# orybkin/video-gcp

Measured on AMD Instinct MI355X. Metric: predicted frames/sec, 64x64x3 seq_len=80 gcp_tree (posterior forward + all loss terms, model(inputs) and model.loss() of train.py:157-159, batch-stat BatchNorm), higher is better.
Workload: dtype f32 (encoder / decoder convs and the tree GEMMs from 512 rows: split-f16 MFMA with f32 accumulate, f32-equivalent; everything else exact f32 MFMA)

## Files before the change

### include/gcpx.h

```cpp
#ifndef GCPX_H
#define GCPX_H

#include <stdint.h>

#ifdef __cplusplus
extern "C" {
#endif

#define GCPX_VERSION 1

typedef enum gcpx_status {
    GCPX_OK = 0,
    GCPX_ERR_INVALID_ARG = -1,
    GCPX_ERR_UNSUPPORTED = -2,
    GCPX_ERR_HIP = -3,
    GCPX_ERR_COMM = -4
} gcpx_status;

typedef enum gcpx_act { GCPX_ACT_NONE = 0, GCPX_ACT_LRELU = 1, GCPX_ACT_TANH = 2 } gcpx_act;

int gcpx_version(void);
const char* gcpx_last_error(void);
int gcpx_conv_grid(void);

// ... 16 lines not shown
    GCPX_HEAD_DLM_NLL_GRAD = 5
} gcpx_head_mode;

typedef struct gcpx_conv_args {
    gcpx_conv_src src[2];
    int32_t nsrc;
    int32_t F;
    int32_t Hin, Win;
    int32_t Hout, Wout;
    int32_t Cin;
    int32_t Cout;
    int32_t out_pitch;
    int32_t upsample;
    int32_t out_act;
    int32_t head_mode;
    const float* wpk;
    const float* bias;
    float* out;
    float* images;
    float* stats_partial;
    const int32_t* raw_row_map;
    const int32_t* src_row_map;
    const int32_t* src_row_frames;
    int32_t n_src_rows;
    int32_t w_split_log2;
    const void* wpk_split;
    const int32_t* w_split_log2_dev;
    int32_t split_layout;
    int32_t nll_rows;
    const float* nll_target;
    float* nll_partial;
    const float* nll_row_weight;
    float nll_scale;
    int32_t _pad3;
    float* images_rows;
    int64_t images_rows_dup;
    const float* bwd_r;
    const float *bwd_scale, *bwd_shift, *bwd_mean, *bwd_rstd;
    const float* addend;
    int32_t addend_frame_div;
    int32_t _pad4;
} gcpx_conv_args;

typedef enum gcpx_split_layout { GCPX_SPLIT_PLAIN = 0, GCPX_SPLIT_ROWFOLD = 1, GCPX_SPLIT_HEAD32 = 2, GCPX_SPLIT_ROWFOLD16 = 3,
                                 GCPX_SPLIT_LOWRES = 4 } gcpx_split_layout;

int gcpx_conv3x3(const gcpx_conv_args* a, void* stream);
int gcpx_conv3x3_grid(const gcpx_conv_args* a);
int gcpx_conv3x3_lowres_supported(const gcpx_conv_args* a);
int gcpx_conv4x4s2(const gcpx_conv_args* a, void* stream);
int gcpx_conv4x4s2_grid(void);
int gcpx_conv4x4s2_image(const float* x, const float* wpk, const float* bias, float* out,
                         int32_t F, int32_t Hin, int32_t Win, int32_t Cout, int32_t out_act, void* stream);

int gcpx_bn_finalize(const float* partial, int32_t n_partial, int32_t pitch, int32_t C, double count,
                     const float* gamma, const float* beta, float eps, float* scale, float* shift,
                     float* running_mean, float* running_var, float momentum, float* mean_out, float* rstd_out,
                     void* stream);
int gcpx_randn(float* out, int64_t n, uint64_t* state, void* stream);
int gcpx_bn_fold(const float* running_mean, const float* running_var, const float* gamma, const float* beta,
                 float eps, int32_t C, float* scale, float* shift, void* stream);

typedef struct gcpx_row_src {
    const float* ptr;
    const int32_t* rowidx;
    const float* scale;
    const float* shiftv;
    int64_t sb, sr;
    int32_t width;
    int32_t shift;
    int32_t act;
    int32_t cmod;
} gcpx_row_src;

typedef enum gcpx_gemm_epi {
    GCPX_EPI_NONE = 0,
    GCPX_EPI_LRELU = 1,
    GCPX_EPI_LSTM = 2,
    GCPX_EPI_GAUSS_SAMPLE = 3
} gcpx_gemm_epi;

struct gcpx_lstm_bwd_args;
typedef struct gcpx_gemm_args {
    gcpx_row_src src[6];
    int32_t nsrc;
    int32_t M, N, K, rpb;
    const float* wpk;
    const float* bias;
    float* out;
    int64_t ob, orow;
    int32_t epi;
    int32_t nbatch;
    float* stats_partial;
    const float* c_prev;
    int64_t c_prev_stride;
    float* h_out;
    float* c_out;
    int64_t hb, hrow;
    float* h_copy;
    int64_t z_src_off, z_w_off, z_bias_off, z_out_off;
    float* gates_out;
    const void* wpk_split;
    const int32_t* w_split_log2_dev;
    int32_t w_split_log2;
    int32_t _pad_split;
    void* x_planes;
// ... 541 lines not shown
```

### video-gcp_amd/forward_plan.py

```python
import ctypes as C
import os
from contextlib import contextmanager

import torch

from . import packing as pk
from . import runtime as rt
from .hparams import GCPHParams
from .params import init_params, encoder_layers, encoder_skip_layers, decoder_layers
from .plan_ops import _Plan, _addr, N_LANES


class ForwardPlanMixin:

    def _plan_encoder(self, plan, tag, x_ptr, F, out_ptr, out_ob, out_orow, out_rpb):
        hp, P, lib = self._hp, self.pk, self.lib
        G = lib.gcpx_conv4x4s2_grid()
        S = hp.img_sz
        skip_idx = encoder_skip_layers(hp)
        skips = {}
        a0 = self._buf(f"{tag}.a0", (F, S // 2, S // 2, hp.ngf))
        enc_rec = dict(F=F, x_ptr=x_ptr, a0=a0, r={}, out=(out_ptr, out_ob, out_orow, out_rpb))
        plan.rec[f"enc:{tag}"] = enc_rec
        plan.add(f"enc.input:{tag}", lib.gcpx_conv4x4s2_image, x_ptr, P["enc.input.w"].data_ptr(),
                 P["enc.input.b"].data_ptr(), a0.data_ptr(), F, S, S, hp.ngf, rt.ACT_LRELU)
        prev = (a0.data_ptr(), hp.ngf, 1, None, None, rt.ACT_NONE)
        if 0 in skip_idx:
            skips[0] = (a0, hp.ngf, None, None, rt.ACT_NONE)
        res = S // 2
        for li, (name, cin, cout, norm) in enumerate(self._enc_layers[1:], start=1):
            r = self._buf(f"{tag}.r{li}", (F, res // 2, res // 2, cout))
            enc_rec["r"][li] = r
            stats = self._buf(f"{tag}.st{li}", (G, 2, cout)) if self.training else None
            a = self._conv_args([prev], F, res, res, res // 2, res // 2, cout, cout, P[f"enc.{name}.w"],
                                P[f"enc.{name}.b"], r, stats=stats)
            self._set_split(a, f"enc.{name}")
            plan.keep.append(a)
            plan.add(f"enc.{name}:{tag}", lib.gcpx_conv4x4s2, C.byref(a))
            res //= 2
            scale, shift = self._bn(plan, f"{tag}.bn{li}", f"encoder.net.{name}.norm", cout, stats, G, cout,
                                    F * res * res)
            prev = (r.data_ptr(), cout, 1, scale, shift, rt.ACT_LRELU)
            if li in skip_idx:
                skips[li] = (r, cout, scale, shift, rt.ACT_LRELU)
        assert res == 4
        ctop = self._c_top
        src = self._rowsrc(prev[0], 16 * ctop, 16 * ctop, 16 * ctop, scale=prev[3], shiftv=prev[4], act=prev[5], cmod=ctop)
        src.sb, src.sr = out_rpb * 16 * ctop, 16 * ctop
        self._gemm(plan, f"enc.head:{tag}", [src], F, hp.nz_enc, out_rpb, P["enc.head.w"], P["enc.head.b"],
                   out=out_ptr, ob=out_ob, orow=out_orow)
        return skips

    def _plan_seq_encoder(self, plan, tag, prefix, enc_traj, out, B):
        hp, P, lib = self._hp, self.pk, self.lib
        T, nz = hp.max_seq_len, hp.nz_enc
        y1 = self._buf(f"{tag}.y1", (B * T, hp.nz_mid))
        y2 = self._buf(f"{tag}.y2", (B * T, hp.nz_mid))
        taps = lambda t, w, **kw: [self._rowsrc(t.data_ptr(), T * w, w, w, shift=d, **kw) for d in (-1, 0, 1)]
        self._gemm(plan, f"{tag}.input", taps(enc_traj, nz), B * T, hp.nz_mid, T, P[f"{tag}.input.w"], P[f"{tag}.input.b"],
                   out=y1.data_ptr(), ob=T * hp.nz_mid, orow=hp.nz_mid, epi=rt.EPI_LRELU)
        assert hp.conv_inf_enc_layers == 1
        nrb = lib.gcpx_gemm_row_blocks(B * T, hp.nz_mid)
        st = self._buf(f"{tag}.st", (nrb, 2, hp.nz_mid)) if self.training else None
        self._gemm(plan, f"{tag}.pyramid-0", taps(y1, hp.nz_mid), B * T, hp.nz_mid, T, P[f"{tag}.pyramid-0.w"],
                   P[f"{tag}.pyramid-0.b"], out=y2.data_ptr(), ob=T * hp.nz_mid, orow=hp.nz_mid, stats=st)
        sc, sh = self._bn(plan, f"{tag}.bn", f"{prefix}.net.pyramid-0.norm", hp.nz_mid, st, nrb, hp.nz_mid, B * T)
        self._gemm(plan, f"{tag}.head", taps(y2, hp.nz_mid, scale=sc, shiftv=sh, act=rt.ACT_LRELU, cmod=hp.nz_mid),
                   B * T, nz, T, P[f"{tag}.head.w"], P[f"{tag}.head.b"], out=out.data_ptr(), ob=T * nz, orow=nz)

    def _plan_attention(self, plan, l, W, el, er, M, n, B, Kp, Vp, tin):
        hp, lib = self._hp, self.lib
        T, nz, dk = hp.max_seq_len, hp.nz_enc, hp.nz_attn_key
        li = l if hp.untied_layers else 0
        qin = self._buf(f"attn.qin{l}", (M, dk))
        self._mlp(plan, f"attn.query{l}", W["attn.query"], [el, er], M, n, out=qin.data_ptr(), ob=n * dk, orow=dk)
        dense = lambda t, w: self._rowsrc(t.data_ptr(), 0, w, w)
        qp = self._buf(f"attn.q{l}", (M, dk))
        self._gemm(plan, f"attn.q_proj{l}", [dense(qin, dk)], M, dk, M, W["attn.q_proj.w"], W["attn.q_proj.b"],
                   out=qp.data_ptr(), ob=0, orow=dk)
        o = self._buf(f"attn.o{l}", (M, nz))
        gamma = self._buf(f"attn.gamma{l}", (M, T))
        temp = self.sd[f"tree_module.tree_modules.{li}.inference.attention.attention_layers.0.temperature"]
        plan.add(f"attn{l}", lib.gcpx_attention, qp.data_ptr(), _addr(Kp, li * B * T * dk), _addr(Vp, li * B * T * nz), None,
                 tin["end_ind"].data_ptr(), temp.data_ptr(), o.data_ptr(), gamma.data_ptr(), M, n, T, dk, nz, hp.n_attention_heads)
        raw = self._buf(f"attn.raw{l}", (M, nz))
        self._gemm(plan, f"attn.out_proj{l}", [dense(o, nz)], M, nz, M, W["attn.out_proj.w"], W["attn.out_proj.b"],
                   out=raw.data_ptr(), ob=0, orow=nz)
        et = self._buf(f"attn.e_tilde{l}", (M, nz))
        self._gemm(plan, f"attn.out{l}", [dense(raw, nz)], M, nz, M, W["attn.out.w"], W["attn.out.b"], out=et.data_ptr(), ob=0, orow=nz)
        plan.rec.setdefault("gamma", {})[l] = gamma
        plan.rec.setdefault("e_tilde", {})[l] = et
# ... 64 lines not shown
    def _build_plan(self, key, tin):
        hp, P, lib = self._hp, self.pk, self.lib
        B, has_traj, has_z, sample_prior, phase, pred_len = key.B, key.has_traj, key.has_z, key.sample_prior, key.phase, key.pred_len
        train_aux = has_traj and phase == "train" and not sample_prior
        L, T, N = hp.hierarchy_levels, hp.max_seq_len, hp.n_nodes
        nz, nv, H, SD = hp.nz_enc, hp.nz_vae, hp.nz_mid_lstm, hp.lstm_state_dim
        PS = 2 ** L + 1
        plan = _Plan(lib)
        G = lib.gcpx_conv_grid()
        def plan_aux_indices():
            AUXK = ("inv_t0", "inv_t1", "cost_start_idx", "cost_end_idx")
            plan.add("aux_sample_indices", lib.gcpx_aux_sample_indices_gauss, tin["end_ind"].data_ptr(), tin["aux_n"].data_ptr(), B,
                     hp.inv_mdl_temp_dist, *[tin[k].data_ptr() for k in AUXK])
        if "aux_n" in tin and pred_len:
            plan_aux_indices()

        E = self._buf("E", (B, PS, nz))
        Hid = self._buf("Hid", (B, PS, SD))
        Z = self._buf("Z", (B, PS, nv))
        PZ = self._buf("PZ", (B, PS, 2 * nv))
        QZ = self._buf("QZ", (B, PS, 2 * nv))
        node_t = self._buf("node_t", (B, N), torch.int32)
        leave = self._buf("leave", (B, N), torch.int32)
        f2n = self._buf("frame2node", (B, T), torch.int32)
        etrow = self._buf("etilde_row", (B * N,), torch.int32)
        seq_len = self._buf("seq_len", (B,), torch.int32)
        kept_idx = self._buf("kept_idx", (B, T), torch.int32)
        node2row = self._buf("node2row", (B, N), torch.int32)

        adaptive, attentive = hp.adaptive, hp.attentive_inference
        if adaptive:
            kept_idx = self._buf("kept_idx", (B, N), torch.int32)
        def plan_bookkeeping():
            if not adaptive:
                plan.add("balanced_binding", lib.gcpx_balanced_binding, tin["end_ind"].data_ptr(), B, L, T, node_t.data_ptr(),
                         leave.data_ptr(), f2n.data_ptr(), etrow.data_ptr(), seq_len.data_ptr(), node2row.data_ptr())
                plan.add("compact_index", lib.gcpx_compact_index, leave.data_ptr(), B, N, T, kept_idx.data_ptr())
                r2f = self._buf("row2frame", (B * T,), torch.int32)
                if self._head_grad_fused(key) or self._rows_direct(key):
                    plan.add("row2frame", lib.gcpx_index_inverse, node2row.data_ptr(), B * N, r2f.data_ptr(), B * T)
                if self._head_grad_fused(key):
                    S_ = hp.img_sz
                    dMD = self._buf("bw.dMD", (B * T, S_, S_, self._head_pitch))
                    plan.add("zero_unmapped", lib.gcpx_zero_unmapped_rows, dMD.data_ptr(), S_ * S_ * self._head_pitch, r2f.data_ptr(), B * T)

        enc_traj = inf_enc = None
        plan.fork([1, 2])
        traj_first = os.environ.get("GCPX_ENC_ORDER") != "small_first"
        def plan_traj_encoder():
            nonlocal enc_traj, inf_enc
            plan.lane = 0
            if has_traj:
                enc_traj = self._buf("enc_traj", (B * T, nz))
                self._plan_encoder(plan, "traj", tin["traj_seq"].data_ptr(), B * T, enc_traj.data_ptr(), T * nz, nz, T)
                if hp.seq_enc == "none":
                    inf_enc = enc_traj
                else:
                    inf_enc = self._buf("inf_enc_seq", (B * T, nz))
                    self._plan_seq_encoder(plan, "seq", "inf_encoder", enc_traj, inf_enc, B)
                if attentive:
                    dk = hp.nz_attn_key
                    n_mod = L if hp.untied_layers else 1
                    if hp.seq_enc == "none":
                        kenc = enc_traj
                    else:
                        kenc = self._buf("inf_key_enc", (B * T, nz))
                        self._plan_seq_encoder(plan, "kseq", "inf_key_encoder.0", enc_traj, kenc, B)
                    keys = self._buf("inf_enc_key_seq", (B * T, dk))
                    dense = lambda t, w: self._rowsrc(t.data_ptr(), 0, w, w)
                    self._gemm(plan, "kseq.key", [dense(kenc, nz)], B * T, dk, B * T, P["kseq.key.w"], P["kseq.key.b"],
                               out=keys.data_ptr(), ob=0, orow=dk)
                    Kp = self._buf("attn.K", (n_mod, B * T, dk))
                    Vp = self._buf("attn.V", (n_mod, B * T, nz))
                    self._gemm(plan, "attn.k_proj", [dense(keys, dk)], B * T, dk, B * T, P["attn.k_proj.w"], P["attn.k_proj.b"],
                               out=Kp.data_ptr(), ob=0, orow=dk, batch=(n_mod, 0, P["attn.k_proj.w"][0].numel(), dk, B * T * dk))
                    self._gemm(plan, "attn.v_proj", [dense(inf_enc, nz)], B * T, nz, B * T, P["attn.v_proj.w"], P["attn.v_proj.b"],
                               out=Vp.data_ptr(), ob=0, orow=nz, batch=(n_mod, 0, P["attn.v_proj.w"][0].numel(), nz, B * T * nz))
                    plan.rec["attn_kv"] = dict(Kp=Kp, Vp=Vp, keys=keys, kenc=kenc, n_mod=n_mod)

        if traj_first:
            plan_traj_encoder()
        plan.lane = 1
        if "rng_all" in tin:
            plan.add("randn", lib.gcpx_randn, tin["rng_all"].data_ptr(), tin["rng_all"].numel(), self._buf("rng_state", (2,), torch.int64).data_ptr())
            if "aux_n" in tin and not pred_len:
                plan.wait(2, 1)
        skips = self._plan_encoder(plan, "I0", tin["I_0"].data_ptr(), B, _addr(E), PS * nz, 0, 1)
        plan.lane = 2
        if not pred_len:
            if "aux_n" in tin:
                plan_aux_indices()
            plan_bookkeeping()
        if hp.attach_cost_mdl and hp.run_cost_mdl and train_aux and self._has_aux_training:
            gt = self._buf("cost_target", (B,))
            rows = hp.input_nc * hp.img_sz
            plan.add("path_cost", lib.gcpx_path_cost, tin["traj_seq"].data_ptr(), tin["cost_start_idx"].data_ptr(),
                     tin["cost_end_idx"].data_ptr(), B, T, rows, hp.img_sz, self._buf("cost_partial", (B, rows)).data_ptr(), gt.data_ptr())
        self._plan_encoder(plan, "Ig", tin["I_g"].data_ptr(), B, _addr(E, 2 ** L * nz), PS * nz, 0, 1)
        outs = {}
        e0 = lambda: self._rowsrc(_addr(E), PS * nz, 0, nz)
        eg = lambda: self._rowsrc(_addr(E, 2 ** L * nz), PS * nz, 0, nz)
        if hp.regress_length and not pred_len:
            plan.wait(2, 1)
            logits = self._buf("seq_len_logits", (B, T))
            self._mlp(plan, "length_pred", P["length_pred"], [e0(), eg()], B, 1, out=logits.data_ptr(), ob=T, orow=0)
            outs["seq_len_logits"] = logits
        if not traj_first:
            plan_traj_encoder()
        plan.lane = 0
        plan.join([1, 2])

        if hp.regress_length and pred_len:
            logits = self._buf("seq_len_logits", (B, T))
            self._mlp(plan, "length_pred", P["length_pred"], [e0(), eg()], B, 1, out=logits.data_ptr(), ob=T, orow=0)
            outs["seq_len_logits"] = logits
            plan.add("sample_length", lib.gcpx_sample_length, logits.data_ptr(), tin["len_u"].data_ptr(), B, T, 2, tin["end_ind"].data_ptr())
            plan_bookkeeping()

        side_merge = False
        for l in range(L):
            W = P[f"tree{l if hp.untied_layers else 0}"]
            s = 2 ** (L - 1 - l)
            n = 2 ** l
            M = B * n
            nodeoff = lambda w: s * w
            el = lambda: self._rowsrc(_addr(E), PS * nz, 2 * s * nz, nz)
            er = lambda: self._rowsrc(_addr(E, 2 * s * nz), PS * nz, 2 * s * nz, nz)
            pz_out = (_addr(PZ, nodeoff(2 * nv)), PS * 2 * nv, 2 * s * 2 * nv)
            z_map = (_addr(Z, nodeoff(nv)), PS * nv, 2 * s * nv)
            nl = hp.n_lstm_layers
            merged = self._buf(f"merged{l}", (M, 2 * nl * H))

            def plan_merge(lv=l, group=None):
                s_, n_ = 2 ** (L - 1 - lv), 2 ** lv
                Wl = P[f"tree{lv if hp.untied_layers else 0}"]
                mg = self._buf(f"merged{lv}", (B * n_, 2 * nl * H))
                if hp.tree_lstm == "sum":
                    for side, mode in ((0, 0), (2 * s_ * SD, 1)):
                        plan.add(f"merge{lv}.{mode}", lib.gcpx_rows_strided, _addr(mg), n_ * SD, SD, _addr(Hid, side), PS * SD, 2 * s_ * SD,
                                 B, n_, SD, mode)
                    return
                if hp.tree_lstm == "linear":
                    h1 = self._rowsrc(_addr(Hid), PS * SD, 2 * s_ * SD, SD)
                    h2 = self._rowsrc(_addr(Hid, 2 * s_ * SD), PS * SD, 2 * s_ * SD, SD)
                    self._gemm(plan, f"merge{lv}", [h1, h2], B * n_, SD, n_, Wl["proj.w"], Wl["proj.b"], out=_addr(mg), ob=n_ * SD, orow=SD,
                               group=group)
                    return
                h1 = self._rowsrc(_addr(Hid), PS * SD, 2 * s_ * SD, H)
                h2 = self._rowsrc(_addr(Hid, 2 * s_ * SD), PS * SD, 2 * s_ * SD, H)
                self._gemm(plan, f"merge{lv}", [h1, h2], B * n_, H, n_, Wl["proj.w"], Wl["proj.b"], out=_addr(mg),
                           ob=n_ * 2 * nl * H, orow=2 * nl * H, batch=(2 * nl, H, Wl["proj.w"][0].numel(), H, H), group=group)
# ... 319 lines not shown
```

### video-gcp_amd/runtime.py

```python
import ctypes as C
import os

_HERE = os.path.dirname(os.path.abspath(__file__))
LIB_PATH = os.path.join(_HERE, "libgcpx.so")

ACT_NONE, ACT_LRELU, ACT_TANH = 0, 1, 2
HEAD_RAW, HEAD_DLM_MEAN, HEAD_DLM_BOTH, HEAD_TANH_NCHW, HEAD_DLM_NLL, HEAD_DLM_NLL_GRAD = 0, 1, 2, 3, 4, 5
SPLIT_PLAIN, SPLIT_ROWFOLD, SPLIT_HEAD32, SPLIT_ROWFOLD16, SPLIT_LOWRES = 0, 1, 2, 3, 4
EPI_NONE, EPI_LRELU, EPI_LSTM, EPI_GAUSS_SAMPLE = 0, 1, 2, 3
GEMM_FORM_TILE, GEMM_FORM_SPLIT_K, GEMM_FORM_SPLIT_F16, GEMM_FORM_PLANES = 0, 1, 2, 3
MLP_PLAIN, MLP_GAUSS, MLP_TANH = 0, 1, 2

vp = C.c_void_p
i32 = C.c_int32
i64 = C.c_int64


class ConvSrc(C.Structure):
    _fields_ = [("ptr", vp), ("scale", vp), ("shift", vp), ("C", i32), ("frame_div", i32), ("act", i32), ("_pad", i32)]


class ConvArgs(C.Structure):
    _fields_ = [("src", ConvSrc * 2), ("nsrc", i32), ("F", i32), ("Hin", i32), ("Win", i32), ("Hout", i32),
                ("Wout", i32), ("Cin", i32), ("Cout", i32), ("out_pitch", i32), ("upsample", i32), ("out_act", i32),
# ... 61 lines not shown

class LstmBwdArgs(C.Structure):
    _fields_ = [("gates", vp), ("c_prev", vp), ("c_new", vp), ("dh_dense", vp), ("dh_pos", vp), ("dc_pos", vp),
                ("dgates", vp), ("dc_prev", vp), ("c_prev_stride", i64), ("pb", i64), ("prow", i64), ("dh_stride", i64),
                ("dcp_stride", i64), ("M", i32), ("H", i32), ("rpb", i32), ("_pad", i32)]


class TreeAccumSrc(C.Structure):
    _fields_ = [("ptr", vp), ("ld", i64), ("off_left", i32), ("off_right", i32), ("off_ctx0", i32), ("off_ctxg", i32),
                ("dst_col", i32), ("_pad", i32)]


class TreeAccumArgs(C.Structure):
    _fields_ = [("src", TreeAccumSrc * 6), ("dst", vp), ("dst_sb", i64), ("slot_stride", i64), ("nsrc", i32), ("B", i32),
                ("n", i32), ("width", i32)]


class ActBwdArgs(C.Structure):
    _fields_ = [("da", vp), ("add", vp), ("r", vp), ("scale", vp), ("shift", vp), ("mean", vp), ("rstd", vp), ("dy", vp),
                ("stats_partial", vp), ("ldc", i64), ("c_off", i32), ("up", i32), ("fsum", i32), ("act", i32), ("F", i32),
                ("H", i32), ("W", i32), ("C", i32)]


class PanelTile(C.Structure):
    _fields_ = [("kind", i32), ("src", i32), ("index", i32), ("length", i32), ("flags", i32), ("nb", i32), ("nf", i32),
                ("h", i32), ("w", i32), ("tile_w", i32), ("n0", i32), ("n_b", i32), ("n_f", i32), ("r0", i32), ("r_b", i32),
                ("r_f", i32), ("c0", i32), ("c_b", i32), ("c_f", i32), ("index_off", i32), ("index_stride", i32),
                ("index_count", i32), ("fill", C.c_float), ("_pad", i32), ("off", i64), ("s_b", i64), ("s_f", i64), ("s_c", i64),
                ("s_y", i64)]


class TrajLayer(C.Structure):
    _fields_ = [("states", vp), ("s_n", i64), ("s_p", i64), ("s_d", i64), ("len", vp), ("dim_t", vp), ("color", C.c_float * 3),
                ("len_i64", i32), ("K", i32), ("P", i32)]


PANEL_MAX_SRCS = 16
PANEL_IMAGE, PANEL_GREY, PANEL_GREY_ADD, PANEL_FILL = 0, 1, 2, 3
PANEL_RESCALE, PANEL_LENGTH_STRICT, PANEL_INDEX_FRAME, PANEL_INDEX_I64, PANEL_LENGTH_I64 = 1, 2, 4, 8, 16

WG_ROWS, WG_CONV1D, WG_CONV3X3, WG_CONV4X4S2 = 0, 1, 2, 3
WMAP_LINEAR, WMAP_CONV, WMAP_CONVT = 0, 1, 2

SYMBOLS = [
    ("gcpx_version", C.c_int, []),
    ("gcpx_last_error", C.c_char_p, []),
    ("gcpx_conv_grid", C.c_int, []),
    ("gcpx_conv3x3", C.c_int, [C.POINTER(ConvArgs), vp]),
    ("gcpx_conv3x3_grid", C.c_int, [C.POINTER(ConvArgs)]),
    ("gcpx_conv3x3_lowres_supported", C.c_int, [C.POINTER(ConvArgs)]),
    ("gcpx_conv4x4s2", C.c_int, [C.POINTER(ConvArgs), vp]),
    ("gcpx_conv4x4s2_grid", C.c_int, []),
    ("gcpx_conv4x4s2_image", C.c_int, [vp, vp, vp, vp, i32, i32, i32, i32, i32, vp]),
    ("gcpx_bn_finalize", C.c_int, [vp, i32, i32, i32, C.c_double, vp, vp, C.c_float, vp, vp, vp, vp, C.c_float, vp, vp, vp]),
    ("gcpx_bn_fold", C.c_int, [vp, vp, vp, vp, C.c_float, i32, vp, vp, vp]),
    ("gcpx_randn", C.c_int, [vp, i64, vp, vp]),
    ("gcpx_gemm", C.c_int, [C.POINTER(GemmArgs), vp]),
    ("gcpx_gemm_row_blocks", C.c_int, [i32, i32]),
    ("gcpx_gemm_form", C.c_int, [C.POINTER(GemmArgs), vp]),
    ("gcpx_gemm_planes_workspace", C.c_int, [i32, i32, i32, vp, vp]),
    ("gcpx_mlp", C.c_int, [C.POINTER(MlpArgs), vp]),
    ("gcpx_balanced_binding", C.c_int, [vp, i32, i32, i32, vp, vp, vp, vp, vp, vp, vp]),
    ("gcpx_dlm_nll", C.c_int, [vp, vp, vp, vp, i32, i32, i32, i32, vp]),
    ("gcpx_gauss_nll", C.c_int, [vp, vp, vp, vp, i32, i32, vp]),
    ("gcpx_kl_gauss", C.c_int, [vp, vp, i32, i32, i32, i64, i64, C.c_float, vp, i64, vp, vp]),
    ("gcpx_gauss_sample", C.c_int, [vp, i64, i64, vp, i64, i64, vp, i64, i64, i32, i32, i32, vp]),
    ("gcpx_seq_index", C.c_int, [vp, i32, i32, vp, vp, vp]),
    ("gcpx_fill_zero", C.c_int, [vp, i64, vp]),
    ("gcpx_copy_rows", C.c_int, [vp, vp, i32, i32, i64, i64, i64, vp]),
    ("gcpx_loss_combine", C.c_int, [C.POINTER(LossArgs), vp]),
    ("gcpx_loss_pre", C.c_int, [C.POINTER(LossArgs), vp, vp, i32, i32, i64, i64, C.c_float, vp, i64, vp, vp]),
    ("gcpx_loss_final", C.c_int, [C.POINTER(LossArgs), vp]),
    ("gcpx_gather_rows", C.c_int, [vp, vp, vp, i32, i32, i32, i32, i64, vp]),
    ("gcpx_gather_rows_rest", C.c_int, [vp, vp, vp, i32, i32, i32, i32, i64, vp, vp]),
    ("gcpx_compact_index", C.c_int, [vp, i32, i32, i32, vp, vp]),
    ("gcpx_seq_pairs", C.c_int, [vp, vp, vp, vp, i32, i32, i32, vp]),
    ("gcpx_rollout_cost", C.c_int, [vp, i64, vp, vp, i64, vp, i32, i32, i32, i32, i32, C.c_float, vp]),
    ("gcpx_masked_row_sum", C.c_int, [vp, vp, vp, i32, i32, vp]),
    ("gcpx_wgrad", C.c_int, [C.POINTER(WgradArgs), vp]),
    ("gcpx_wgrad_classify", C.c_int, [C.POINTER(WgradArgs), i32, C.POINTER(C.c_int32), C.POINTER(C.c_int32)]),
    ("gcpx_wgrad_group", C.c_int, [vp, vp, i32, i32, i32, vp]),
    ("gcpx_wgrad_conv3x3", C.c_int, [vp, i32, vp, i32, i32, i32, i32, i32, vp, i32, vp]),
    ("gcpx_wgrad_conv3x3_split", C.c_int, [vp, i32, vp, i32, i32, i32, i32, i32, vp, i32, vp]),
    ("gcpx_wgrad_conv3x3_split_up", C.c_int, [vp, i32, C.POINTER(ConvArgs), i32, vp, i32, vp]),
    ("gcpx_wgrad_conv3x3_split_src", C.c_int, [vp, i32, vp, vp, vp, vp, i32, i32, i32, i32, i32, vp, vp, i32, vp]),
    ("gcpx_wgrad_image4x4s2", C.c_int, [vp, vp, vp, vp, i32, i32, vp, i32, vp]),
    ("gcpx_split_pack_group", C.c_int, [vp, i32, vp]),
    ("gcpx_split_pack_group2", C.c_int, [vp, i32, vp, vp]),
    ("gcpx_wgrad_reduce", C.c_int, [vp, i32, i32, i32, vp, i32, i32, i32, i32, vp, i64, i32, i32, vp]),
    ("gcpx_colsum", C.c_int, [vp, i64, i32, i32, i32, i64, i32, vp, vp, vp, i32, vp]),
    ("gcpx_reduce_partials", C.c_int, [vp, i32, i64, i32, vp, i32, vp]),
    ("gcpx_lstm_bwd", C.c_int, [C.POINTER(LstmBwdArgs), vp]),
    ("gcpx_mlp_bwd", C.c_int, [C.POINTER(MlpBwdArgs), vp]),
    ("gcpx_mlp_bwd_group", C.c_int, [C.POINTER(MlpBwdArgs), i32, vp]),
    ("gcpx_mlp_bwd_blocks", C.c_int, [i32]),
    ("gcpx_gn_lrelu_bwd", C.c_int, [vp, vp, vp, vp, vp, vp, i32, i32, i32, C.c_float, C.c_float, vp]),
    ("gcpx_gn_bwd_blocks", C.c_int, [i32]),
    ("gcpx_tanh_bwd_rows", C.c_int, [vp, vp, vp, i64, i64, i32, i32, i32, vp]),
    ("gcpx_lrelu_bwd", C.c_int, [vp, vp, vp, i64, C.c_float, vp]),
    ("gcpx_kl_bwd", C.c_int, [vp, vp, vp, vp, i32, i32, i32, i64, i64, C.c_float, C.c_float, vp]),
    ("gcpx_kl_bwd_weighted", C.c_int, [vp, vp, vp, vp, i32, i32, i32, i64, i64, C.c_float, C.c_float, vp, i64, vp]),
    ("gcpx_kl_bwd_scheduled", C.c_int, [vp, vp, vp, vp, i32, i32, i32, i64, i64, C.c_float, C.c_float, vp, i64, vp, vp]),
    ("gcpx_rows_strided", C.c_int, [vp, i64, i64, vp, i64, i64, i32, i32, i32, i32, vp]),
    ("gcpx_latent_bwd", C.c_int, [vp, vp, vp, i64, i64, vp, i64, i64, vp, i64, vp, i64, vp, vp, i32, i32, i32, vp]),
    ("gcpx_tree_accum", C.c_int, [C.POINTER(TreeAccumArgs), vp]),
    ("gcpx_timestep_scatter", C.c_int, [vp, i64, i64, vp, vp, i32, i32, i32, i32, vp]),
# ... 145 lines not shown
```

### video-gcp_amd/sequential.py

```python
import ctypes as C
import os

import torch

from . import runtime as rt
from .model import GCPTreeModel, Outputs, _Plan, _addr
from .params import init_params_sequential


class GCPSequentialModel(GCPTreeModel):
    _has_aux_training = True
    _has_pred_length = False
    _rng_in_plan = False
    _has_training = True

    def _check_hp(self, hp):
        assert hp.lstm_init in ("zero", "mlp")
        assert hp.n_actions <= 16 or not hp.action_conditioned_pred, "the action rows are padded to one 16-column k-group"

    @property
    def _nets(self):
        return ("gen_lstm",) if self._hp.deterministic else ("prior_lstm", "inf_lstm", "gen_lstm")

    def _default_params(self, hp, seed):
# ... 107 lines not shown
            stages.append(lambda g: self._gemm(plan, f"{name}.embed", srcs, B, H, 1, W["embed.w"], W["embed.b"],
                                               out=xs_buf[0].data_ptr(), ob=H, orow=0, group=g))
        for i in range(nl):
            def layer(g, i=i):
                s_in, s_out = state[par][i], state[1 - par][i]
                xs = self._rowsrc(xs_buf[i].data_ptr(), H, 0, H)
                hs = self._rowsrc(s_in.data_ptr(), 2 * H, 0, H)
                lstm = (_addr(s_in, H), 2 * H, s_out.data_ptr(), _addr(s_out, H), 2 * H, 0, xs_buf[i + 1].data_ptr())
                if i == 0 and fused:
                    self._gemm(plan, f"{name}.lstm0", list(srcs) + [hs], B, 4 * H, 1, W[w0 + ".w"], W[w0 + ".b"], epi=rt.EPI_LSTM,
                               lstm=lstm, group=g)
                else:
                    self._gemm(plan, f"{name}.lstm{i}", [xs, hs], B, 4 * H, 1, W[f"lstm{i}.w"], W[f"lstm{i}.b"], epi=rt.EPI_LSTM,
                               lstm=lstm, group=g)
            stages.append(layer)
        stages.append(lambda g: self._gemm(plan, f"{name}.out", [self._rowsrc(xs_buf[nl].data_ptr(), H, 0, H)], B, N_out, 1,
                                           W["out.w"], W["out.b"], out=out_ptr, ob=out_ob, orow=0, group=g))
        return stages

    def _plan_hsp(self, plan, name, W, srcs, B, state, par, out_ptr, out_ob, N_out):
        for st in self._hsp_stages(plan, name, W, srcs, B, state, par, out_ptr, out_ob, N_out):
            st(None)

    def _build_plan(self, key, tin):
        hp, P, lib = self._hp, self.pk, self.lib
        B, has_traj, has_z, sample_prior, phase, with_loss = key.B, key.has_traj, key.has_z, key.sample_prior, key.phase, key.with_loss
        T, nz, nv, H, nl = hp.max_seq_len, hp.nz_enc, hp.nz_vae, hp.nz_mid_lstm, hp.n_lstm_layers
        S = hp.img_sz
        plan = _Plan(lib)
        X = self._buf("seq.X", (B, T, nz))
        EG = self._buf("seq.EG", (B, nz))
        PZ = self._buf("seq.PZ", (B, T - 1, 2 * nv))
        QZ = self._buf("seq.QZ", (B, T - 1, 2 * nv), zero=True)
        Z = self._buf("seq.Z", (B, T - 1, nv))
        idx = self._buf("seq.idx", (B, T), torch.int32)
        seq_len = self._buf("seq.len", (B,), torch.int32)
        plan.add("seq_index", lib.gcpx_seq_index, tin["end_ind"].data_ptr(), B, T, idx.data_ptr(), seq_len.data_ptr())
        train_aux = has_traj and phase == "train" and not sample_prior
        if "aux_n" in tin:
            AUXK = ("inv_t0", "inv_t1", "cost_start_idx", "cost_end_idx")
            plan.add("aux_sample_indices", lib.gcpx_aux_sample_indices_gauss, tin["end_ind"].data_ptr(), tin["aux_n"].data_ptr(), B,
                     hp.inv_mdl_temp_dist, *[tin[k].data_ptr() for k in AUXK])

        enc_traj = None
        plan.fork([1, 2])
        plan.lane = 1
        skips = self._plan_encoder(plan, "I0", tin["I_0"].data_ptr(), B, _addr(X), T * nz, 0, 1)
        plan.lane = 2
        if hp.attach_cost_mdl and hp.run_cost_mdl and train_aux and "cost_start_idx" in tin:
            rows = hp.input_nc * hp.img_sz
            plan.add("path_cost", lib.gcpx_path_cost, tin["traj_seq"].data_ptr(), tin["cost_start_idx"].data_ptr(),
                     tin["cost_end_idx"].data_ptr(), B, T, rows, hp.img_sz, self._buf("cost_partial", (B, rows)).data_ptr(),
                     self._buf("cost_target", (B,)).data_ptr())
        self._plan_encoder(plan, "Ig", tin["I_g"].data_ptr(), B, _addr(EG), nz, 0, 1)
        plan.lane = 0
        if has_traj:
            enc_traj = self._buf("enc_traj", (B * T, nz))
            self._plan_encoder(plan, "traj", tin["traj_seq"].data_ptr(), B * T, enc_traj.data_ptr(), T * nz, nz, T)
        plan.join([1, 2])
        outs = {}
        e0 = lambda: self._rowsrc(_addr(X), T * nz, 0, nz)
        eg = lambda: self._rowsrc(_addr(EG), nz, 0, nz)
        if hp.regress_length:
            logits = self._buf("seq_len_logits", (B, T))
            self._mlp(plan, "length_pred", P["length_pred"], [e0(), eg()], B, 1, out=logits.data_ptr(), ob=T, orow=0)
            outs["seq_len_logits"] = logits

        EA = None
        if hp.action_conditioned_pred:
            na = hp.n_actions
            assert tuple(tin["actions"].shape) == (B, T - 1, na), "actions [B, T-1, n_actions]: action t leads to frame t + 1 (sequential.py:50)"
            A16 = self._buf("seq.actions16", (B, T - 1, 16), zero=True)
            plan.add("actions.pad", lib.gcpx_rows_strided, A16.data_ptr(), (T - 1) * 16, 16, tin["actions"].data_ptr(), (T - 1) * na, na,
                     B, T - 1, na, 0)
            EA = self._buf("seq.EA", (B, T - 1, nz))
            self._mlp(plan, "action_encoder", P["action_encoder"], [self._rowsrc(A16.data_ptr(), (T - 1) * 16, 16, 16)], B * (T - 1), T - 1,
                      out=EA.data_ptr(), ob=(T - 1) * nz, orow=nz)

        NETS = self._nets
        keep = self.save_for_backward
        if keep:
            Sall = {net: self._buf(f"{net}.S", (T, nl, B, 2 * H)) for net in NETS}
            XSall = {net: self._buf(f"{net}.XS", (T - 1, nl + 1, B, H)) for net in NETS}
            plan.rec["seq"] = dict(S=Sall, XS=XSall, X=X, EG=EG, PZ=PZ, QZ=QZ, Z=Z, EA=EA)
            for net in NETS:
                plan.add(f"zero.{net}", lib.gcpx_fill_zero, Sall[net].data_ptr(), nl * B * 2 * H * 4)

            class _StepState:
                def __init__(self, S, t):
                    self.S, self.t = S, t

                def __getitem__(self, par):
                    tt = self.t if par == (self.t & 1) else self.t + 1
                    return [self.S[tt, i] for i in range(nl)]
            state_of = lambda net, t: _StepState(Sall[net], t)
            xs_of = lambda net, t: [XSall[net][t, i] for i in range(nl + 1)]
        else:
            state = {net: [[self._buf(f"{net}.s{par}.{i}", (B, 2 * H)) for i in range(nl)] for par in range(2)] for net in NETS}
            for net in state:
                for i in range(nl):
                    plan.add(f"zero.{net}.{i}", lib.gcpx_fill_zero, state[net][0][i].data_ptr(), B * 2 * H * 4)
            state_of = lambda net, t: state[net]
            xs_of = lambda net, t: None
        def ctx(t):
            c = [e0(), eg()] if hp.context_every_step else []
            return c + ([self._rowsrc(_addr(EA, t * nz), (T - 1) * nz, 0, nz)] if EA is not None else [])
        posterior = has_traj and not sample_prior and not has_z and not hp.deterministic
        xt_of = lambda t: self._rowsrc(_addr(X, t * nz), T * nz, 0, nz)

        def prior_stages(t):
            return self._hsp_stages(plan, f"prior{t}", P["prior_lstm"], [xt_of(t)] + ctx(t), B, state_of("prior_lstm", t), t & 1,
# ... 310 lines not shown
```

Before: 504,300.

## Fuse encoder input conv with first strided conv in one LDS-resident kernel

Adds a kernel that computes the 64x64 image input conv (f32 MFMA) into LDS, then splits the activation into two f16 parts per frame and runs the second 4x4 stride-2 conv with split-f16 MFMA, writing BN stats partials. The goal is to avoid writing the 32x32x16 first-layer activation to global memory and reading it back, and to save one launch, for encoders whose skips are not read. It uses about 140 KB of LDS per block and half the usual grid, so occupancy drops. It also adds a per-frame scaling step for the f16 split.

```diff
diff --git a/include/gcpx.h b/include/gcpx.h
--- a/include/gcpx.h
+++ b/include/gcpx.h
@@ -92,6 +92,10 @@
 int gcpx_conv4x4s2_grid(void);
 int gcpx_conv4x4s2_image(const float* x, const float* wpk, const float* bias, float* out,
                          int32_t F, int32_t Hin, int32_t Win, int32_t Cout, int32_t out_act, void* stream);
+int gcpx_conv4x4s2_image_fused(const float* x, const float* w0pk, const float* bias0, int32_t act0, float* a0_out,
+                               const gcpx_conv_args* a, void* stream);
+int gcpx_conv4x4s2_image_fused_supported(const gcpx_conv_args* a, int32_t Himg, int32_t Wimg);
+int gcpx_conv4x4s2_image_fused_grid(void);
 
 int gcpx_bn_finalize(const float* partial, int32_t n_partial, int32_t pitch, int32_t C, double count,
                      const float* gamma, const float* beta, float eps, float* scale, float* shift,
diff --git a/video-gcp_amd/csrc/conv_enc_fused.hip b/video-gcp_amd/csrc/conv_enc_fused.hip
--- /dev/null
+++ b/video-gcp_amd/csrc/conv_enc_fused.hip
@@ -0,0 +1,274 @@
+#include "common.h"
+
+#include <cstdlib>
+
+namespace {
+
+typedef _Float16 h8 __attribute__((ext_vector_type(8)));
+
+__device__ __forceinline__ f32x4 mfma32h(h8 a, h8 b, f32x4 c) {
+    return __builtin_amdgcn_mfma_f32_16x16x32_f16(a, b, c, 0, 0, 0);
+}
+
+struct EncFusedCfg {
+    static constexpr int HIMG = 64, HIN = 32, HOUT = 16, CIN = 16, COUT = 32, CT = 2;
+    static constexpr int WP = 2, WC = 2, PGW = 8, NSTEP = 8;
+    static constexpr int PIXB = CIN * 4 + 16, FRAME_PIX = HIN * HIN, FRAME_BYTES = FRAME_PIX * PIXB;
+    static constexpr int PITCH = HIMG + 8, ROWS = HIMG + 2, PLANE = ROWS * PITCH, IMG_BYTES = 3 * PLANE * 4;
+    static constexpr int RED_BYTES = WP * 2 * COUT * 4;
+    static constexpr int LDS_BYTES = FRAME_BYTES + IMG_BYTES + RED_BYTES;
+    static constexpr int F4 = 3 * HIMG * HIMG / 4, NPF = F4 / 256;
+    static_assert(FRAME_BYTES == 81920 && IMG_BYTES == 57024 && F4 % 256 == 0 && LDS_BYTES <= 160 * 1024, "layout");
+};
+
+template <bool A0, bool STATS>
+__global__ void __launch_bounds__(256) conv4x4s2_image_fused_kernel(const float* __restrict__ x, const float* __restrict__ w0pk,
+                                                                    const float* __restrict__ bias0, const int act0,
+                                                                    float* __restrict__ a0_out, const gcpx_conv_args a, const int nrows) {
+    using Cfg = EncFusedCfg;
+    constexpr int HIMG = Cfg::HIMG, HIN = Cfg::HIN, HOUT = Cfg::HOUT, COUT = Cfg::COUT, CT = Cfg::CT, WP = Cfg::WP, PGW = Cfg::PGW;
+    constexpr int PIXB = Cfg::PIXB, FRAME_PIX = Cfg::FRAME_PIX, NSTEP = Cfg::NSTEP, PITCH = Cfg::PITCH, PLANE = Cfg::PLANE;
+    constexpr int F4 = Cfg::F4, NPF = Cfg::NPF;
+    extern __shared__ float4 encf_smem4[];
+    char* lds = reinterpret_cast<char*>(encf_smem4);
+    float* img = reinterpret_cast<float*>(lds + Cfg::FRAME_BYTES);
+    float* red = reinterpret_cast<float*>(lds + Cfg::FRAME_BYTES + Cfg::IMG_BYTES);
+    float* wmax = reinterpret_cast<float*>(lds + Cfg::CIN * 4);
+    const int tid = threadIdx.x, lane = tid & 63, wave = tid >> 6;
+    const int wp = wave % WP, wc = wave / WP;
+    const int j = lane & 15, q = lane >> 4;
+    const int F = a.F, G = gridDim.x;
+    const float slope0 = act0 == GCPX_ACT_LRELU ? 0.2f : 1.f, slope1 = a.out_act == GCPX_ACT_LRELU ? 0.2f : 1.f;
+
+    for (int i = tid; i < 3 * 2 * PITCH; i += 256) {
+        const int pl = i / (2 * PITCH), r = (i / PITCH) % 2, c = i % PITCH;
+        img[pl * PLANE + (r ? HIMG + 1 : 0) * PITCH + c] = 0.f;
+    }
+    for (int i = tid; i < 3 * Cfg::ROWS * 2; i += 256) {
+        const int pl = i / (Cfg::ROWS * 2), r = (i / 2) % Cfg::ROWS, c = (i & 1) ? HIMG + 4 : 3;
+        img[pl * PLANE + r * PITCH + c] = 0.f;
+    }
+    if (STATS && tid < 2 * COUT)
+        for (int r = F + (int)blockIdx.x; r < nrows; r += G) a.stats_partial[(size_t)r * 2 * COUT + tid] = 0.f;
+
+    float w0[12];
+#pragma unroll
+    for (int t = 0; t < 12; ++t) w0[t] = w0pk[t * 64 + lane];
+    const float4 bv0 = *reinterpret_cast<const float4*>(bias0 + q * 4);
+    h8 w1[NSTEP][2];
+    {
+        const char* wbase = reinterpret_cast<const char*>(a.wpk_split) + (size_t)wc * 2048 + lane * 16;
+#pragma unroll
+        for (int s = 0; s < NSTEP; ++s) {
+            w1[s][0] = *reinterpret_cast<const h8*>(wbase + (size_t)s * CT * 2048);
+            w1[s][1] = *reinterpret_cast<const h8*>(wbase + (size_t)s * CT * 2048 + 1024);
+        }
+    }
+    const int c1 = wc * 16 + q * 4;
+    const float4 bv1 = *reinterpret_cast<const float4*>(a.bias + c1);
+    const int ew = a.w_split_log2_dev ? __builtin_amdgcn_readfirstlane(*a.w_split_log2_dev) : a.w_split_log2;
+
+    int base[PGW], pin_[PGW];
+    unsigned vmask[PGW];
+#pragma unroll
+    for (int pt = 0; pt < PGW; ++pt) {
+        const int pin = (wp + pt * WP) * 16 + j;
+        const int oy = pin / HOUT, ox = pin % HOUT;
+        pin_[pt] = pin;
+        base[pt] = ((2 * oy - 1) * HIN + 2 * ox - 1) * PIXB;
+        unsigned m = 0;
+        for (int k = 0; k < 4; ++k) {
+            if (2 * oy - 1 + k >= 0 && 2 * oy - 1 + k < HIN) m |= 1u << k;
+            if (2 * ox - 1 + k >= 0 && 2 * ox - 1 + k < HIN) m |= 16u << k;
+        }
+        vmask[pt] = m;
+    }
+
+    auto img_off = [&](const int i) __attribute__((always_inline)) {
+        const int pl = i / (HIMG * HIMG / 4), rem = i % (HIMG * HIMG / 4);
+        const int y = rem / (HIMG / 4), x4 = rem % (HIMG / 4);
+        return pl * PLANE + (y + 1) * PITCH + 4 + 4 * x4;
+    };
+    const f32x4* x4p = reinterpret_cast<const f32x4*>(x);
+    __builtin_amdgcn_s_waitcnt(0x0f70);
+
+    for (int f = blockIdx.x; f < F; f += G) {
+        {
+            const f32x4* src = x4p + (size_t)f * F4;
+            f32x4 v[NPF];
+#pragma unroll
+            for (int k = 0; k < NPF; ++k) v[k] = src[k * 256 + tid];
+#pragma unroll
+            for (int k = 0; k < NPF; ++k) *reinterpret_cast<f32x4*>(img + img_off(k * 256 + tid)) = v[k];
+        }
+        __syncthreads();
+
+        float amax = 0.f;
+#pragma unroll
+        for (int gi = 0; gi < FRAME_PIX / 64; gi += 4) {
+            float b[4][12];
+#pragma unroll
+            for (int u = 0; u < 4; ++u) {
+                const int p = ((gi + u) * 4 + wave) * 16 + j;
+                const int oy = p / HIN, ox = p % HIN;
+                const float* bp = img + (2 * oy) * PITCH + 3 + 2 * ox + q;
+#pragma unroll
+                for (int ci = 0; ci < 3; ++ci)
+#pragma unroll
+                    for (int ky = 0; ky < 4; ++ky) b[u][ci * 4 + ky] = bp[ci * PLANE + ky * PITCH];
+            }
+            f32x4 acc[4];
+#pragma unroll
+            for (int u = 0; u < 4; ++u) acc[u] = f32x4{0, 0, 0, 0};
+#pragma unroll
+            for (int t = 0; t < 12; ++t)
+#pragma unroll
+                for (int u = 0; u < 4; ++u) acc[u] = mfma16(w0[t], b[u][t], acc[u]);
+#pragma unroll
+            for (int u = 0; u < 4; ++u) {
+                const int p = ((gi + u) * 4 + wave) * 16 + j;
+                f32x4 v = acc[u];
+                v[0] += bv0.x; v[1] += bv0.y; v[2] += bv0.z; v[3] += bv0.w;
+                v[0] = lrelu(v[0], slope0); v[1] = lrelu(v[1], slope0); v[2] = lrelu(v[2], slope0); v[3] = lrelu(v[3], slope0);
+                *reinterpret_cast<f32x4*>(lds + p * PIXB + 16 * q) = v;
+                if constexpr (A0) *reinterpret_cast<f32x4*>(a0_out + ((size_t)f * FRAME_PIX + p) * 16 + q * 4) = v;
+                amax = fmaxf(amax, fmaxf(fmaxf(fabsf(v[0]), fabsf(v[1])), fmaxf(fabsf(v[2]), fabsf(v[3]))));
+            }
+        }
+#pragma unroll
+        for (int m = 1; m < 64; m <<= 1) amax = fmaxf(amax, __shfl_xor(amax, m));
+        if (lane == 0) wmax[wave] = amax;
+        __syncthreads();
+        amax = fmaxf(fmaxf(wmax[0], wmax[1]), fmaxf(wmax[2], wmax[3]));
+        int ex = 14 + 127 - (int)((__float_as_uint(amax) >> 23) & 0xff);
+        ex = __builtin_amdgcn_readfirstlane(amax > 0.f ? max(-100, min(min(100, 126 - ew), ex)) : min(100, 126 - ew));
+        const float sx2 = __uint_as_float((unsigned)(127 + ex) << 23);
+#pragma unroll
+        for (int i = tid; i < FRAME_PIX * 2; i += 256) {
+            const int c8 = i % 2, pix = i / 2;
+            char* p = lds + pix * PIXB + 32 * c8;
+            const float4 v0 = *reinterpret_cast<const float4*>(p), v1 = *reinterpret_cast<const float4*>(p + 16);
+            const float fv[8] = {v0.x * sx2, v0.y * sx2, v0.z * sx2, v0.w * sx2, v1.x * sx2, v1.y * sx2, v1.z * sx2, v1.w * sx2};
+            h8 p1, p2;
+#pragma unroll
+            for (int e = 0; e < 8; ++e) {
+                p1[e] = (_Float16)fv[e];
+                p2[e] = (_Float16)fmaf((float)p1[e], -1.f, fv[e]);
+            }
+            *reinterpret_cast<h8*>(p) = p1;
+            *reinterpret_cast<h8*>(p + 16) = p2;
+        }
+        __syncthreads();
+
+        f32x4 acc[PGW];
+#pragma unroll
+        for (int pt = 0; pt < PGW; ++pt) acc[pt] = f32x4{0, 0, 0, 0};
+        auto load_b = [&](const int step, h8 (&b)[PGW][2]) __attribute__((always_inline)) {
+            const int tap = 2 * step + (q >> 1), grp = q & 1;
+            const int ky = tap >> 2, kx = tap & 3;
+            const int tapoff = (ky * HIN + kx) * PIXB + grp * 32;
+#pragma unroll
+            for (int pt = 0; pt < PGW; ++pt) {
+                const bool ok = ((vmask[pt] >> ky) & 1u) && ((vmask[pt] >> (4 + kx)) & 1u);
+                const char* p = lds + (ok ? base[pt] + tapoff : 0);
+                const h8 t0 = *reinterpret_cast<const h8*>(p), t1 = *reinterpret_cast<const h8*>(p + 16);
+                const h8 z = {0, 0, 0, 0, 0, 0, 0, 0};
+                b[pt][0] = ok ? t0 : z;
+                b[pt][1] = ok ? t1 : z;
+            }
+        };
+        auto mm = [&](const int step, const h8 (&b)[PGW][2]) __attribute__((always_inline)) {
+#pragma unroll
+            for (int pt = 0; pt < PGW; ++pt) acc[pt] = mfma32h(w1[step][1], b[pt][0], acc[pt]);
+#pragma unroll
+            for (int pt = 0; pt < PGW; ++pt) acc[pt] = mfma32h(w1[step][0], b[pt][1], acc[pt]);
+#pragma unroll
+            for (int pt = 0; pt < PGW; ++pt) acc[pt] = mfma32h(w1[step][0], b[pt][0], acc[pt]);
+        };
+        h8 bA[PGW][2], bB[PGW][2];
+        load_b(0, bA);
+#pragma unroll
+        for (int step = 0; step < NSTEP; step += 2) {
+            load_b(step + 1, bB);
+            mm(step, bA);
+            if (step + 2 < NSTEP) load_b(step + 2, bA);
+            mm(step + 1, bB);
+        }
+        const float inv = __uint_as_float((unsigned)(127 - ex - ew) << 23);
+        f32x4 st1 = f32x4{0, 0, 0, 0}, st2 = f32x4{0, 0, 0, 0};
+#pragma unroll
+        for (int pt = 0; pt < PGW; ++pt) {
+            float* op = a.out + ((size_t)f * HOUT * HOUT + pin_[pt]) * COUT;
+            f32x4 v = acc[pt];
+            v[0] = fmaf(v[0], inv, bv1.x); v[1] = fmaf(v[1], inv, bv1.y); v[2] = fmaf(v[2], inv, bv1.z); v[3] = fmaf(v[3], inv, bv1.w);
+            v[0] = lrelu(v[0], slope1); v[1] = lrelu(v[1], slope1); v[2] = lrelu(v[2], slope1); v[3] = lrelu(v[3], slope1);
+            *reinterpret_cast<f32x4*>(op + c1) = v;
+            if constexpr (STATS) {
+                st1 += v;
+#pragma unroll
+                for (int r = 0; r < 4; ++r) st2[r] = fmaf(v[r], v[r], st2[r]);
+            }
+        }
+        if constexpr (STATS) {
+#pragma unroll
+            for (int r = 0; r < 4; ++r) {
+                const float s1 = row16_sum(st1[r]);
+                const float s2 = row16_sum(st2[r]);
+                if (j == 0) {
+                    red[(wp * 2 + 0) * COUT + c1 + r] = s1;
+                    red[(wp * 2 + 1) * COUT + c1 + r] = s2;
+                }
+            }
+        }
+        __syncthreads();
+        if (STATS && tid < 2 * COUT) {
+            const int which = tid / COUT, c = tid % COUT;
+            float sum = 0.f;
+#pragma unroll
+            for (int w_ = 0; w_ < WP; ++w_) sum += red[(w_ * 2 + which) * COUT + c];
+            a.stats_partial[((size_t)f * 2 + which) * COUT + c] = sum;
+        }
+    }
+}
+
+bool fused_shape_ok(const gcpx_conv_args* a, int Himg, int Wimg) {
+    return a && Himg == 64 && Wimg == 64 && a->nsrc == 1 && a->src[0].frame_div == 1 && a->src[0].C == 16 && !a->src[0].scale &&
+           !a->src[0].shift && a->src[0].act == GCPX_ACT_NONE && a->Cin == 16 && a->Cout == 32 && a->out_pitch == 32 && a->Hin == 32 &&
+           a->Win == 32 && a->Hout == 16 && a->Wout == 16 && a->wpk_split && a->split_layout == GCPX_SPLIT_PLAIN && a->F > 0 &&
+           a->F <= gcpx_conv4x4s2_grid() && !a->src_row_map && !a->addend;
+}
+
+}
+
+extern "C" int gcpx_conv4x4s2_image_fused_grid(void) { return gcpx_conv_grid() / 2; }
+
+extern "C" int gcpx_conv4x4s2_image_fused_supported(const gcpx_conv_args* a, int32_t Himg, int32_t Wimg) {
+    return fused_shape_ok(a, Himg, Wimg) ? 1 : 0;
+}
+
+extern "C" int gcpx_conv4x4s2_image_fused(const float* x, const float* w0pk, const float* bias0, int32_t act0, float* a0_out,
+                                          const gcpx_conv_args* a, void* stream_) {
+    hipStream_t stream = reinterpret_cast<hipStream_t>(stream_);
+    GCPX_CHECK_ARG(a != nullptr && x && w0pk && bias0, "null pointer");
+    GCPX_CHECK_ARG(fused_shape_ok(a, 64, 64), "not a problem gcpx_conv4x4s2_image_fused_supported accepts");
+    GCPX_CHECK_ARG(a->bias && a->out, "null bias / out");
+    GCPX_CHECK_ARG(act0 == GCPX_ACT_NONE || act0 == GCPX_ACT_LRELU, "act0 must be NONE or LRELU");
+    using Cfg = EncFusedCfg;
+    const int form = (a0_out ? 1 : 0) + (a->stats_partial ? 2 : 0);
+    const auto kern = form == 0 ? conv4x4s2_image_fused_kernel<false, false> : form == 1 ? conv4x4s2_image_fused_kernel<true, false>
+                    : form == 2 ? conv4x4s2_image_fused_kernel<false, true> : conv4x4s2_image_fused_kernel<true, true>;
+    static bool attr_set[4] = {false, false, false, false};
+    if (!attr_set[form]) {
+        hipError_t e = hipFuncSetAttribute(reinterpret_cast<const void*>(kern), hipFuncAttributeMaxDynamicSharedMemorySize, Cfg::LDS_BYTES);
+        if (e != hipSuccess) {
+            gcpx_set_error("conv4x4s2 image (fused): hipFuncSetAttribute(%d B): %s", Cfg::LDS_BYTES, hipGetErrorString(e));
+            return GCPX_ERR_HIP;
+        }
+        attr_set[form] = true;
+    }
+    int grid = gcpx_conv4x4s2_image_fused_grid();
+    if (grid > a->F) grid = a->F;
+    hipLaunchKernelGGL(kern, dim3(grid), dim3(256), Cfg::LDS_BYTES, stream, x, w0pk, bias0, act0, a0_out, *a, gcpx_conv4x4s2_grid());
+    GCPX_CHECK_LAUNCH();
+    return GCPX_OK;
+}
diff --git a/video-gcp_amd/forward_plan.py b/video-gcp_amd/forward_plan.py
--- a/video-gcp_amd/forward_plan.py
+++ b/video-gcp_amd/forward_plan.py
@@ -13,30 +13,52 @@
 
 class ForwardPlanMixin:
 
-    def _plan_encoder(self, plan, tag, x_ptr, F, out_ptr, out_ob, out_orow, out_rpb):
+    def _plan_encoder(self, plan, tag, x_ptr, F, out_ptr, out_ob, out_orow, out_rpb, skips_read=True):
         hp, P, lib = self._hp, self.pk, self.lib
         G = lib.gcpx_conv4x4s2_grid()
         S = hp.img_sz
         skip_idx = encoder_skip_layers(hp)
         skips = {}
-        a0 = self._buf(f"{tag}.a0", (F, S // 2, S // 2, hp.ngf))
-        enc_rec = dict(F=F, x_ptr=x_ptr, a0=a0, r={}, out=(out_ptr, out_ob, out_orow, out_rpb))
+        enc_rec = dict(F=F, x_ptr=x_ptr, a0=None, r={}, out=(out_ptr, out_ob, out_orow, out_rpb))
         plan.rec[f"enc:{tag}"] = enc_rec
-        plan.add(f"enc.input:{tag}", lib.gcpx_conv4x4s2_image, x_ptr, P["enc.input.w"].data_ptr(),
-                 P["enc.input.b"].data_ptr(), a0.data_ptr(), F, S, S, hp.ngf, rt.ACT_LRELU)
-        prev = (a0.data_ptr(), hp.ngf, 1, None, None, rt.ACT_NONE)
-        if 0 in skip_idx:
+        a0_read = (0 in skip_idx and skips_read) or self.save_for_backward
+        name1, _, cout1, _ = self._enc_layers[1]
+        r1 = self._buf(f"{tag}.r1", (F, S // 4, S // 4, cout1))
+        st1 = self._buf(f"{tag}.st1", (G, 2, cout1)) if self.training else None
+        a1 = self._conv_args([(None, hp.ngf, 1, None, None, rt.ACT_NONE)], F, S // 2, S // 2, S // 4, S // 4, cout1, cout1,
+                             P[f"enc.{name1}.w"], P[f"enc.{name1}.b"], r1, stats=st1)
+        self._set_split(a1, f"enc.{name1}")
+        plan.keep.append(a1)
+        fused = (os.environ.get("GCPX_NO_ENC_FUSE") is None and (not skips_read or os.environ.get("GCPX_ENC_FUSE_ALL") is not None) and
+                 bool(lib.gcpx_conv4x4s2_image_fused_supported(C.byref(a1), S, S)))
+        a0 = self._buf(f"{tag}.a0", (F, S // 2, S // 2, hp.ngf)) if a0_read or not fused else None
+        enc_rec["a0"] = a0
+        if a0 is not None:
+            a1.src[0].ptr = a0.data_ptr()
+        if fused:
+            plan.add(f"enc.input+{name1}:{tag}", lib.gcpx_conv4x4s2_image_fused, x_ptr, P["enc.input.w"].data_ptr(),
+                     P["enc.input.b"].data_ptr(), rt.ACT_LRELU, a0.data_ptr() if a0 is not None else None, C.byref(a1))
+        else:
+            plan.add(f"enc.input:{tag}", lib.gcpx_conv4x4s2_image, x_ptr, P["enc.input.w"].data_ptr(),
+                     P["enc.input.b"].data_ptr(), a0.data_ptr(), F, S, S, hp.ngf, rt.ACT_LRELU)
+        prev = None
+        if 0 in skip_idx and a0 is not None:
             skips[0] = (a0, hp.ngf, None, None, rt.ACT_NONE)
         res = S // 2
         for li, (name, cin, cout, norm) in enumerate(self._enc_layers[1:], start=1):
-            r = self._buf(f"{tag}.r{li}", (F, res // 2, res // 2, cout))
+            if li == 1:
+                r, stats = r1, st1
+                if not fused:
+                    plan.add(f"enc.{name}:{tag}", lib.gcpx_conv4x4s2, C.byref(a1))
+            else:
+                r = self._buf(f"{tag}.r{li}", (F, res // 2, res // 2, cout))
+                stats = self._buf(f"{tag}.st{li}", (G, 2, cout)) if self.training else None
+                a = self._conv_args([prev], F, res, res, res // 2, res // 2, cout, cout, P[f"enc.{name}.w"],
+                                    P[f"enc.{name}.b"], r, stats=stats)
+                self._set_split(a, f"enc.{name}")
+                plan.keep.append(a)
+                plan.add(f"enc.{name}:{tag}", lib.gcpx_conv4x4s2, C.byref(a))
             enc_rec["r"][li] = r
-            stats = self._buf(f"{tag}.st{li}", (G, 2, cout)) if self.training else None
-            a = self._conv_args([prev], F, res, res, res // 2, res // 2, cout, cout, P[f"enc.{name}.w"],
-                                P[f"enc.{name}.b"], r, stats=stats)
-            self._set_split(a, f"enc.{name}")
-            plan.keep.append(a)
-            plan.add(f"enc.{name}:{tag}", lib.gcpx_conv4x4s2, C.byref(a))
             res //= 2
             scale, shift = self._bn(plan, f"{tag}.bn{li}", f"encoder.net.{name}.norm", cout, stats, G, cout,
                                     F * res * res)
@@ -207,7 +229,7 @@
             plan.lane = 0
             if has_traj:
                 enc_traj = self._buf("enc_traj", (B * T, nz))
-                self._plan_encoder(plan, "traj", tin["traj_seq"].data_ptr(), B * T, enc_traj.data_ptr(), T * nz, nz, T)
+                self._plan_encoder(plan, "traj", tin["traj_seq"].data_ptr(), B * T, enc_traj.data_ptr(), T * nz, nz, T, skips_read=False)
                 if hp.seq_enc == "none":
                     inf_enc = enc_traj
                 else:
@@ -251,7 +273,7 @@
             rows = hp.input_nc * hp.img_sz
             plan.add("path_cost", lib.gcpx_path_cost, tin["traj_seq"].data_ptr(), tin["cost_start_idx"].data_ptr(),
                      tin["cost_end_idx"].data_ptr(), B, T, rows, hp.img_sz, self._buf("cost_partial", (B, rows)).data_ptr(), gt.data_ptr())
-        self._plan_encoder(plan, "Ig", tin["I_g"].data_ptr(), B, _addr(E, 2 ** L * nz), PS * nz, 0, 1)
+        self._plan_encoder(plan, "Ig", tin["I_g"].data_ptr(), B, _addr(E, 2 ** L * nz), PS * nz, 0, 1, skips_read=False)
         outs = {}
         e0 = lambda: self._rowsrc(_addr(E), PS * nz, 0, nz)
         eg = lambda: self._rowsrc(_addr(E, 2 ** L * nz), PS * nz, 0, nz)
diff --git a/video-gcp_amd/runtime.py b/video-gcp_amd/runtime.py
--- a/video-gcp_amd/runtime.py
+++ b/video-gcp_amd/runtime.py
@@ -137,6 +137,9 @@
     ("gcpx_conv4x4s2", C.c_int, [C.POINTER(ConvArgs), vp]),
     ("gcpx_conv4x4s2_grid", C.c_int, []),
     ("gcpx_conv4x4s2_image", C.c_int, [vp, vp, vp, vp, i32, i32, i32, i32, i32, vp]),
+    ("gcpx_conv4x4s2_image_fused", C.c_int, [vp, vp, vp, i32, vp, C.POINTER(ConvArgs), vp]),
+    ("gcpx_conv4x4s2_image_fused_supported", C.c_int, [C.POINTER(ConvArgs), i32, i32]),
+    ("gcpx_conv4x4s2_image_fused_grid", C.c_int, []),
     ("gcpx_bn_finalize", C.c_int, [vp, i32, i32, i32, C.c_double, vp, vp, C.c_float, vp, vp, vp, vp, C.c_float, vp, vp, vp]),
     ("gcpx_bn_fold", C.c_int, [vp, vp, vp, vp, C.c_float, i32, vp, vp, vp]),
     ("gcpx_randn", C.c_int, [vp, i64, vp, vp]),
diff --git a/video-gcp_amd/sequential.py b/video-gcp_amd/sequential.py
--- a/video-gcp_amd/sequential.py
+++ b/video-gcp_amd/sequential.py
@@ -183,11 +183,11 @@
             plan.add("path_cost", lib.gcpx_path_cost, tin["traj_seq"].data_ptr(), tin["cost_start_idx"].data_ptr(),
                      tin["cost_end_idx"].data_ptr(), B, T, rows, hp.img_sz, self._buf("cost_partial", (B, rows)).data_ptr(),
                      self._buf("cost_target", (B,)).data_ptr())
-        self._plan_encoder(plan, "Ig", tin["I_g"].data_ptr(), B, _addr(EG), nz, 0, 1)
+        self._plan_encoder(plan, "Ig", tin["I_g"].data_ptr(), B, _addr(EG), nz, 0, 1, skips_read=False)
         plan.lane = 0
         if has_traj:
             enc_traj = self._buf("enc_traj", (B * T, nz))
-            self._plan_encoder(plan, "traj", tin["traj_seq"].data_ptr(), B * T, enc_traj.data_ptr(), T * nz, nz, T)
+            self._plan_encoder(plan, "traj", tin["traj_seq"].data_ptr(), B * T, enc_traj.data_ptr(), T * nz, nz, T, skips_read=False)
         plan.join([1, 2])
         outs = {}
         e0 = lambda: self._rowsrc(_addr(X), T * nz, 0, nz)
```

After: 512,700, median of 6. 1.02x the previous value.
